# przemektmalon/SeqALib

Measured on AMD Instinct MI355X. Metric: GCUPS (DP cell updates/s) on batched 4k×4k SW; bit-exact score match, higher is better.
Workload: dtype f16 (integer-exact below 2048); 1 GPU; sw_batch_10000x4096x4096; pairs_per_gpu=10000, total_pairs=10000, m=4096, n=4096, algo=SmithWatermanSA, match=equal<char>, parallelism=pair-shard x1

## Files before the change

seqalib_amd/csrc/sa_traceback_so.hip:

```cpp
#include <limits.h>

#include "sa_internal.h"

namespace sa {

typedef const void __attribute__((address_space(1)))* so_gptr;
typedef void __attribute__((address_space(3)))* so_lptr;

constexpr int kSoOps = 64;
template <int R>
struct SoLds {
    static constexpr int RT = (2 * R + 31) / 32;
    static constexpr int kTags = 0;
    static constexpr int kEdge = kTags + 32 * RT * 256;
    static constexpr int kRowCodes = kEdge + 5 * 1024;
    static constexpr int kColCodes = kRowCodes + ((R + 3) / 4) * 256;
    static constexpr int kOps = kColCodes + 8 * 256;
    static constexpr int kBytes = kOps + kSoOps * 64;
};

__device__ __forceinline__ uint32_t so_code8(uint32_t sp, uint32_t b) {
    return (b == ((sp >> 8) & 255u) ? 8u : 0u) | (b == ((sp >> 16) & 255u) ? 16u : 0u) |
           (b == (sp >> 24) ? 24u : 0u);
}

template <int R>
__global__ __launch_bounds__(64) void traceback_so_kernel(TbParams P) {
    using L = SoLds<R>;
    constexpr int RT = L::RT;
    constexpr int BAND = kWave * R;
    __shared__ __attribute__((aligned(16))) uint8_t s_so[L::kBytes];
    typedef volatile uint8_t __attribute__((address_space(3))) lds_u8;
    typedef volatile uint32_t __attribute__((address_space(3))) lds_u32;
    typedef volatile uint16_t __attribute__((address_space(3))) lds_u16;
    lds_u8* const vb = (lds_u8*)s_so;
    lds_u32* const vw = (lds_u32*)s_so;
    const int lane = threadIdx.x;
    const uint32_t slot = blockIdx.x * blockDim.x + threadIdx.x;
    if (slot >= P.count) return;
    const uint32_t pidx = P.pair_base + slot;
    sa_result res = P.res[pidx];
    if (res.flags & SA_FLAG_BAD_SHAPE) return;
    if (!tb_mine(P, res.flags)) {
        tb_release(P, &P.res[pidx], res.flags);
        return;
    }
    res.flags &= tb_clear_mask(P);
    const uint64_t o1 = P.off1[pidx], o2 = P.off2[pidx];
    const int m = (int)(P.off1[pidx + 1] - o1);
    const int n = (int)(P.off2[pidx + 1] - o2);
    const uint8_t* s1 = P.seq1 + o1;
    const uint8_t* s2 = P.seq2 + o2;
    typedef uint8_t __attribute__((address_space(1))) glb_u8;
    glb_u8* ops = (glb_u8*)(P.ops + o1 + o2 + pidx);
    const uint8_t* const dir = P.dirs + (uint64_t)slot * P.dir_slot;
    const uint64_t band_stride = P.band_stride;
    const uint32_t npk = (uint32_t)(band_stride / (kWave * 16));
    const uint32_t* const sh_base = P.snap_h + (uint64_t)slot * P.snap_h_slot;
    const int32_t* const sp_base = P.snap_p + (uint64_t)slot * P.snap_p_slot;
    const uint32_t snap_nch = P.snap_nch;
    const uint32_t symp = P.prof[4];
    const uint32_t pf0 = P.prof[0], pf1 = P.prof[1], pf2 = P.prof[2], pf3 = P.prof[3];
    uint32_t mt = 0;
#pragma unroll
    for (int a = 0; a < 4; ++a)
#pragma unroll
        for (int b = 0; b < 4; ++b) {
            const uint32_t sa_ = (symp >> (8 * a)) & 255u, sb_ = (symp >> (8 * b)) & 255u;
            const bool v = P.lutbits ? ((P.lutbits[(sa_ << 3) | (sb_ >> 5)] >> (sb_ & 31u)) & 1u) != 0 : sa_ == sb_;
            mt |= (v ? 1u : 0u) << (a * 4 + b);
        }
    const bool allow = P.allow != 0;
    const int G = P.gap, MA = P.match, MI = P.mismatch;
    const uint32_t CU = (uint32_t)(-(4 * G + 2)) & 0xffffu;
    const uint32_t CL = (uint32_t)(4 * G + 1) & 0xffffu;

    uint32_t k = 0, k0 = 0;
    auto emit = [&](uint8_t op) __attribute__((always_inline)) {
        const uint32_t q = k - k0;
        vb[L::kOps + (q >> 2) * 256 + lane * 4 + (q & 3)] = op;
        ++k;
    };
    auto flush = [&]() __attribute__((always_inline)) {
        for (uint32_t q = 0; q < k - k0; ++q) ops[k0 + q] = vb[L::kOps + (q >> 2) * 256 + lane * 4 + (q & 3)];
        k0 = k;
    };

    int wb = -1, wt = 0, wc = 0;
    int cb = 0, ct = 0, cc = 0, cr = 0, cq = 0;
    auto locate = [&](int i, int j) __attribute__((always_inline)) {
        const int ii = i - 1;
        cb = ii / BAND;
        const int rem = ii - cb * BAND;
        ct = rem / R;
        cr = rem - ct * R;
        const int s = j - 1 + ct;
        cc = s >> 5;
        cq = s & 31;
    };
    auto ready = [&](int i, int j) __attribute__((always_inline)) -> bool {
        if (k - k0 >= (uint32_t)kSoOps) return false;
        if (!(i > 0 && j > 0)) return true;
        locate(i, j);
        return cb == wb && ct == wt && cc == wc;
    };
    auto recompute = [&](int i, int j) __attribute__((always_inline)) {
        if (!(i > 0 && j > 0)) return;
        locate(i, j);
        wb = cb; wt = ct; wc = cc;
        const int r0 = cb * BAND + ct * R;
        const int j0 = 32 * cc - ct;
        const bool has_top = !(cb == 0 && ct == 0);
        const int bp = ct > 0 ? cb : cb - 1, tp = ct > 0 ? ct - 1 : kWave - 1;
        const int slo = j0 + tp;
        const int pk0 = slo >> 3;
        if (has_top) {
            const uint8_t* base = dir + (uint64_t)bp * band_stride;
#pragma unroll
            for (int d = 0; d < 5; ++d) {
                const int pk = pk0 + d;
                if (pk >= 0 && (uint32_t)pk < npk)
                    __builtin_amdgcn_global_load_lds((so_gptr)(base + ((uint64_t)pk * kWave + tp) * 16),
                                                     (so_lptr)(s_so + L::kEdge + d * 1024), 16, 0, 0);
            }
        }
        int Hp[R];
        int corner = 0;
        const bool has_left = cc > 0 && j0 >= 1;
        if (has_left) {
            const uint64_t e = (uint64_t)cb * snap_nch + (cc - 1);
            const uint32_t* sh = sh_base + e * (R / 2) * kWave + ct;
#pragma unroll
            for (int q = 0; q < R / 2; ++q) {
                const uint32_t w = sh[q * kWave];
                Hp[2 * q] = (int)(w & 0xffffu) << 2;
                Hp[2 * q + 1] = (int)(w >> 16) << 2;
            }
            if (r0 > 0) corner = (sp_base[e * kWave + ct] & 0xffff) << 2;
        } else {
#pragma unroll
            for (int r = 0; r < R; ++r) Hp[r] = 0;
        }
        uint32_t tab[R];
#pragma unroll
        for (int r = 0; r < R; r += 4) {
            uint32_t cw = 0;
#pragma unroll
            for (int e = 0; e < 4 && r + e < R; ++e) {
                const int row = r0 + r + e;
                const uint32_t c8 = row < m ? so_code8(symp, s1[row]) : 0u;
                tab[r + e] = c8 == 0 ? pf0 : c8 == 8 ? pf1 : c8 == 16 ? pf2 : pf3;
                cw |= c8 << (8 * e);
            }
            vw[(L::kRowCodes >> 2) + (r >> 2) * 64 + lane] = cw;
        }
        const int qlo = j0 < 0 ? -j0 : 0;
        const int qhi = j - 1 - j0;
#pragma unroll
        for (int w = 0; w < 8; ++w) {
            uint32_t cw = 0;
#pragma unroll
            for (int e = 0; e < 4; ++e) {
                const int q = 4 * w + e, jj = j0 + q;
                cw |= (q >= qlo && q <= qhi && jj < n ? so_code8(symp, s2[jj]) : 0u) << (8 * e);
            }
            vw[(L::kColCodes >> 2) + w * 64 + lane] = cw;
        }
        asm volatile("s_waitcnt vmcnt(0)" ::: "memory");
        auto top_of = [&](int q) -> int {
            if (!has_top) return 0;
            const int s = slo + q;
            const int d = (s >> 3) - pk0;
            return (int)((lds_u16*)(s_so + L::kEdge + d * 1024 + lane * 16 + (s & 7) * 2))[0] << 2;
        };
        auto sym_of = [&](int q) -> uint32_t {
            return (vw[(L::kColCodes >> 2) + (q >> 2) * 64 + lane] >> (8 * (q & 3))) & 255u;
        };
        auto put = [&](int q, int r, uint32_t& rec) __attribute__((always_inline)) {
            if ((r & 15) == 15 || r == R - 1) {
                const uint32_t wv = (r & 15) == 15 ? rec : rec >> (32 - 2 * ((r & 15) + 1));
                vw[(q * RT + (r >> 4)) * 64 + lane] = wv;
                rec = 0;
            }
        };
#define SO_CELL(P, HP, HU, DR, REC, TAB, SYM)                                                      \
    "v_add_u16 %[" #P "0], %[cl], %[" HP "]\n\t"                                                  \
    "v_bfe_i32 %[" #P "dn], %[" TAB "], %[" SYM "], 8\n\t"                                         \
    "v_add_u16 %[" #P "dn], %[" HP "], %[" #P "dn]\n\t"                                            \
    "v_sub_u16_e64 %[" #P "1], %[" HU "], %[cu] clamp\n\t"                                         \
    "v_max_i16 %[" #P "0], %[" DR "], %[" #P "0]\n\t"                                              \
    "v_max_i16 %[" #P "0], %[" #P "1], %[" #P "0]\n\t"                                             \
    "v_and_b32 %[" HP "], -4, %[" #P "0]\n\t"                                                      \
    "v_alignbit_b32 %[" REC "], %[" #P "0], %[" REC "], 2\n\t"
#define SO_CELL2                                                                                   \
    "v_add_u16 %[a0], %[cl], %[ha]\n\t"                                                            \
    "v_add_u16 %[b0], %[cl], %[hb]\n\t"                                                            \
    "v_bfe_i32 %[adn], %[taba], %[syma], 8\n\t"                                                    \
    "v_bfe_i32 %[bdn], %[tabb], %[symb], 8\n\t"                                                    \
    "v_add_u16 %[adn], %[ha], %[adn]\n\t"                                                          \
    "v_add_u16 %[bdn], %[hb], %[bdn]\n\t"                                                          \
    "v_sub_u16_e64 %[a1], %[hb], %[cu] clamp\n\t"                                                  \
    "v_sub_u16_e64 %[b1], %[hub], %[cu] clamp\n\t"                                                 \
    "v_max_i16 %[a0], %[da], %[a0]\n\t"                                                            \
    "v_max_i16 %[b0], %[db], %[b0]\n\t"                                                            \
    "v_max_i16 %[a0], %[a1], %[a0]\n\t"                                                            \
    "v_max_i16 %[b0], %[b1], %[b0]\n\t"                                                            \
    "v_and_b32 %[ha], -4, %[a0]\n\t"                                                               \
    "v_and_b32 %[hb], -4, %[b0]\n\t"                                                               \
    "v_alignbit_b32 %[reca], %[a0], %[reca], 2\n\t"                                                \
    "v_alignbit_b32 %[recb], %[b0], %[recb], 2"
        auto column = [&](int q, int top, int ptop) __attribute__((always_inline)) {
            const uint32_t sym = sym_of(q);
            uint32_t dcur;
            asm("v_bfe_i32 %0, %1, %2, 8\n\tv_add_u16 %0, %3, %0" : "=&v"(dcur) : "v"(tab[0]), "v"(sym), "v"(ptop));
            uint32_t hu = (uint32_t)top, rec = 0;
#pragma unroll
            for (int r = 0; r < R; ++r) {
                uint32_t a0, a1, adn;
                asm(SO_CELL(a, "hp", "hu", "dr", "rec", "tabn", "sym")
                    : [a0] "=&v"(a0), [a1] "=&v"(a1), [adn] "=&v"(adn), [hp] "+v"(Hp[r]), [rec] "+v"(rec)
                    : [dr] "v"(dcur), [hu] "v"(hu), [cu] "s"(CU), [cl] "s"(CL),
                      [tabn] "v"(tab[r + 1 < R ? r + 1 : r]), [sym] "v"(sym));
                dcur = adn;
                hu = (uint32_t)Hp[r];
                put(q, r, rec);
            }
        };
        auto column_pair = [&](int q, int topA, int topB, int ptop) __attribute__((always_inline)) {
            const uint32_t symA = sym_of(q), symB = sym_of(q + 1);
            uint32_t da, db;
            asm("v_bfe_i32 %0, %1, %2, 8\n\tv_add_u16 %0, %3, %0" : "=&v"(da) : "v"(tab[0]), "v"(symA), "v"(ptop));
            asm("v_bfe_i32 %0, %1, %2, 8\n\tv_add_u16 %0, %3, %0" : "=&v"(db) : "v"(tab[0]), "v"(symB), "v"(topA));
            uint32_t recA = 0, recB = 0;
            {
                uint32_t a0, a1, adn;
                asm(SO_CELL(a, "hp", "hu", "dr", "rec", "tabn", "sym")
                    : [a0] "=&v"(a0), [a1] "=&v"(a1), [adn] "=&v"(adn), [hp] "+v"(Hp[0]), [rec] "+v"(recA)
                    : [dr] "v"(da), [hu] "v"((uint32_t)topA), [cu] "s"(CU), [cl] "s"(CL),
                      [tabn] "v"(tab[R > 1 ? 1 : 0]), [sym] "v"(symA));
                da = adn;
                put(q, 0, recA);
            }
#pragma unroll
            for (int r = 1; r < R; ++r) {
                const uint32_t hub = r >= 2 ? (uint32_t)Hp[r - 2] : (uint32_t)topB;
                uint32_t a0, a1, adn, b0, b1, bdn;
                asm(SO_CELL2
                    : [a0] "=&v"(a0), [a1] "=&v"(a1), [adn] "=&v"(adn), [b0] "=&v"(b0), [b1] "=&v"(b1),
                      [bdn] "=&v"(bdn), [ha] "+v"(Hp[r]), [hb] "+v"(Hp[r - 1]), [reca] "+v"(recA), [recb] "+v"(recB)
                    : [da] "v"(da), [db] "v"(db), [hub] "v"(hub), [cu] "s"(CU), [cl] "s"(CL),
                      [taba] "v"(tab[r + 1 < R ? r + 1 : r]), [syma] "v"(symA), [tabb] "v"(tab[r]), [symb] "v"(symB));
                da = adn;
                db = bdn;
                put(q, r, recA);
                put(q + 1, r - 1, recB);
            }
            {
                const uint32_t hub = R >= 2 ? (uint32_t)Hp[R - 2] : (uint32_t)topB;
                uint32_t b0, b1, bdn;
                asm(SO_CELL(b, "hp", "hu", "dr", "rec", "tabn", "sym")
                    : [b0] "=&v"(b0), [b1] "=&v"(b1), [bdn] "=&v"(bdn), [hp] "+v"(Hp[R - 1]), [rec] "+v"(recB)
                    : [dr] "v"(db), [hu] "v"(hub), [cu] "s"(CU), [cl] "s"(CL), [tabn] "v"(tab[R - 1]), [sym] "v"(symB));
                put(q + 1, R - 1, recB);
            }
        };
#undef SO_CELL
#undef SO_CELL2
        int ptop = corner;
        int q = qlo;
        for (; q + 1 <= qhi; q += 2) {
            const int ta = top_of(q), tb = top_of(q + 1);
            column_pair(q, ta, tb, ptop);
            ptop = tb;
        }
        if (q == qhi) column(q, top_of(q), ptop);
    };
    auto tag = [&]() __attribute__((always_inline)) -> uint32_t {
        return (vw[(cq * RT + (cr >> 4)) * 64 + lane] >> (2 * (cr & 15))) & 3u;
    };
    auto cell_match = [&]() __attribute__((always_inline)) -> bool {
        const uint32_t a = (vb[L::kRowCodes + (cr >> 2) * 256 + lane * 4 + (cr & 3)] >> 3) & 3u;
        const uint32_t b = (vb[L::kColCodes + (cq >> 2) * 256 + lane * 4 + (cq & 3)] >> 3) & 3u;
        return ((mt >> (a * 4 + b)) & 1u) != 0;
    };

    int i = res.end_i, j = res.end_j, V = res.score;
    if (m == 0 || n == 0) { i = 0; j = 0; }
    bool fin = false, parked = true;
    for (;;) {
        if (__builtin_amdgcn_ballot_w64(!fin && !parked) == 0) {
            if (__builtin_amdgcn_ballot_w64(!fin) == 0) break;
            if (!fin) { flush(); recompute(i, j); parked = false; }
        }
        if (!fin && !parked) {
            if (!(i > 0 && j > 0) || V == 0) {
                fin = true;
            } else if (!ready(i, j)) {
                parked = true;
            } else {
                const uint32_t f = tag();
                const bool dg = f == 3u, up = f == 2u;
                const bool v = dg && cell_match();
                emit(dg ? (v ? 'M' : (allow ? 'S' : 'X')) : (up ? 'U' : 'L'));
                V -= dg ? (v ? MA : MI) : G;
                i -= (dg || up) ? 1 : 0;
                j -= up ? 0 : 1;
            }
        }
    }
    flush();
    res.start_i = i;
    res.start_j = j;
    res.nops = k;
    P.res[pidx] = res;
}

constexpr int kSo4DefaultLp = 4;
#ifdef SA_TB_STATS
__device__ unsigned long long g_so4_stats[8];
extern "C" int sa_debug_so4_stats(unsigned long long* out, int reset) {
    if (hipMemcpyFromSymbol(out, HIP_SYMBOL(g_so4_stats), sizeof(g_so4_stats)) != hipSuccess) return 1;
    if (reset) {
        unsigned long long z[8] = {};
        if (hipMemcpyToSymbol(HIP_SYMBOL(g_so4_stats), z, sizeof(z)) != hipSuccess) return 1;
    }
    return 0;
}
#endif
template <int R, int LP>
struct So4Lds {
    static constexpr int kPairs = kWave / LP;
    static constexpr int kTags = 64;
    static constexpr int kQuad = 1024 + 32;
    static constexpr int kEdge = kTags + kPairs * kQuad;
    static constexpr int kEdge2 = kEdge + 64 * 16;
    static constexpr int kRowC = kEdge2 + (LP < 5 ? 64 * 16 : 0);
    static constexpr int kColC = kRowC + kPairs * 32;
    static constexpr int kBytes = kColC + kPairs * 32;
};

template <int ALG, int R, int LP>
__global__ __launch_bounds__(64) void traceback_so4_kernel(TbParams P) {
    constexpr bool NWK = ALG == SA_NW;
    using L = So4Lds<R, LP>;
    constexpr int RS = R / LP;
    constexpr int BAND = kWave * R;
    static_assert((LP == 4 || LP == 8) && R >= LP && R % LP == 0 && RS <= 16, "LP sublanes of <= 16 rows");
    __shared__ __attribute__((aligned(16))) uint8_t s_so[L::kBytes];
    typedef volatile uint8_t __attribute__((address_space(3))) lds_u8;
    typedef volatile uint32_t __attribute__((address_space(3))) lds_u32;
    typedef volatile uint16_t __attribute__((address_space(3))) lds_u16;
    typedef volatile uint64_t __attribute__((address_space(3))) lds_u64;
    lds_u8* const vb = (lds_u8*)s_so;
    lds_u32* const vw = (lds_u32*)s_so;
    const int lane = threadIdx.x, quad = lane / LP, sub = lane % LP;
    const uint32_t slot = blockIdx.x * L::kPairs + quad;
    bool live = slot < P.count;
    const uint32_t pidx = P.pair_base + (live ? slot : 0);
    sa_result res = P.res[pidx];
    if (live && !(res.flags & SA_FLAG_BAD_SHAPE) && !tb_mine(P, res.flags)) {
        if (sub == 0) tb_release(P, &P.res[pidx], res.flags);
        live = false;
    }
    live = live && !(res.flags & SA_FLAG_BAD_SHAPE);
    if (__builtin_amdgcn_ballot_w64(live) == 0) return;
    res.flags &= tb_clear_mask(P);
    const uint64_t o1 = P.off1[pidx], o2 = P.off2[pidx];
    const int m = (int)(P.off1[pidx + 1] - o1);
    const int n = (int)(P.off2[pidx + 1] - o2);
    const uint8_t* s1 = P.seq1 + o1;
    const uint8_t* s2 = P.seq2 + o2;
    typedef uint8_t __attribute__((address_space(1))) glb_u8;
    glb_u8* ops = (glb_u8*)(P.ops + o1 + o2 + pidx);
    const uint8_t* const dir = P.dirs + (uint64_t)(live ? slot : 0) * P.dir_slot;
    const uint64_t band_stride = P.band_stride;
    const uint32_t npk = (uint32_t)(band_stride / (kWave * 16));
    const uint32_t* const sh_base = P.snap_h + (uint64_t)(live ? slot : 0) * P.snap_h_slot;
    const int32_t* const sp_base = P.snap_p + (uint64_t)(live ? slot : 0) * P.snap_p_slot;
    const uint32_t snap_nch = P.snap_nch;
    const uint32_t symp = P.prof[4];
    const uint32_t pf0 = P.prof[0], pf1 = P.prof[1], pf2 = P.prof[2], pf3 = P.prof[3];
    uint32_t mt = 0;
#pragma unroll
    for (int a = 0; a < 4; ++a)
#pragma unroll
        for (int b = 0; b < 4; ++b) {
            const uint32_t sa_ = (symp >> (8 * a)) & 255u, sb_ = (symp >> (8 * b)) & 255u;
            const bool v = P.lutbits ? ((P.lutbits[(sa_ << 3) | (sb_ >> 5)] >> (sb_ & 31u)) & 1u) != 0 : sa_ == sb_;
            mt |= (v ? 1u : 0u) << (a * 4 + b);
        }
    const bool allow = P.allow != 0;
    const int G = P.gap, MA = P.match, MI = P.mismatch;
    const uint32_t CU = (uint32_t)(NWK ? 4 * G + 2 : -(4 * G + 2)) & 0xffffu;
    const uint32_t CL = (uint32_t)(4 * G + 1) & 0xffffu;
    const int D0 = P.t16_delta;
    auto border = [&](int x) __attribute__((always_inline)) -> int {
        return 4 * (x * G - D0);
    };

    uint32_t k = 0;
    auto emit = [&](uint8_t op) __attribute__((always_inline)) {
        if (sub == 0) ops[k] = op;
        ++k;
    };
    int cb = 0, ct = 0, cc = 0, cr = 0, cq = 0;
    auto locate = [&](int i, int j) __attribute__((always_inline)) {
        const int ii = i - 1;
        cb = ii / BAND;
        const int rem = ii - cb * BAND;
        ct = rem / R;
        cr = rem - ct * R;
        const int s = j - 1 + ct;
        cc = s >> 5;
        cq = s & 31;
    };
    uint64_t rowc = 0, colc = 0;
    auto pack_codes = [&](int base) __attribute__((always_inline)) -> uint64_t {
        uint64_t c = 0;
#pragma unroll
        for (int d = 0; d < 8; ++d) {
            uint32_t x = (vw[(base >> 2) + d] >> 3) & 0x03030303u;
            x = (x | (x >> 6)) & 0x000f000fu;
            x = (x | (x >> 12)) & 0xffu;
            c |= (uint64_t)x << (8 * d);
        }
        return c;
    };
#ifdef SA_TB_STATS
    unsigned long long st_rounds = 0, st_iters = 0, st_wait = 0, st_sub = 0, st_nsub = 0;
    const unsigned long long st_t0 = __builtin_amdgcn_s_memtime();
    unsigned long long st_a = 0;
#endif
    auto recompute = [&](bool act, int i, int j) __attribute__((always_inline)) {
#ifdef SA_TB_STATS
        st_a = __builtin_amdgcn_s_memtime();
#endif
        int r0 = 0, j0 = 0, qlo = 0, qhi = -1, slo = 0, pk0 = 0, bp = 0, tp = 0;
        bool has_top = false, has_left = false;
        if (act) {
            locate(i, j);
            r0 = cb * BAND + ct * R;
            j0 = 32 * cc - ct;
            qlo = j0 < 0 ? -j0 : 0;
            qhi = j - 1 - j0;
            has_top = !(cb == 0 && ct == 0);
            bp = ct > 0 ? cb : cb - 1;
            tp = ct > 0 ? ct - 1 : kWave - 1;
            slo = j0 + tp;
            pk0 = slo >> 3;
            has_left = cc > 0 && j0 >= 1;
            if (has_top) {
                const uint8_t* base = dir + (uint64_t)bp * band_stride;
                const int pk = pk0 + sub;
                if (sub < 5 && pk >= 0 && (uint32_t)pk < npk)
                    __builtin_amdgcn_global_load_lds((so_gptr)(base + ((uint64_t)pk * kWave + tp) * 16),
                                                     (so_lptr)(s_so + L::kEdge), 16, 0, 0);
                if constexpr (LP < 5) {
                    const int pk4 = pk0 + 4;
                    if (sub == 0 && pk4 >= 0 && (uint32_t)pk4 < npk)
                        __builtin_amdgcn_global_load_lds((so_gptr)(base + ((uint64_t)pk4 * kWave + tp) * 16),
                                                         (so_lptr)(s_so + L::kEdge2), 16, 0, 0);
                }
            }
        }
        int Hp[RS];
        int corner = 0;
        uint32_t tab[RS];
#pragma unroll
        for (int r = 0; r < RS; ++r) { Hp[r] = 0; tab[r] = pf0; }
        if (act) {
            const int rs0 = sub * RS;
            uint32_t w[RS], b1[RS], b2[32 / LP];
            const uint64_t e = has_left ? (uint64_t)cb * snap_nch + (cc - 1) : 0;
            const uint32_t* sh = sh_base + e * (R / 2) * kWave + ct;
#pragma unroll
            for (int r = 0; r < RS; ++r) w[r] = sh[((rs0 + r) >> 1) * kWave];
            const uint32_t wc = sh[(rs0 > 0 ? (rs0 - 1) >> 1 : 0) * kWave];
            const int32_t pc = sp_base[e * kWave + ct];
#pragma unroll
            for (int r = 0; r < RS; ++r) b1[r] = s1[min(r0 + rs0 + r, m - 1)];
#pragma unroll
            for (int x = 0; x < 32 / LP; ++x) b2[x] = s2[min(max(j0 + sub * (32 / LP) + x, 0), n - 1)];
            if constexpr (NWK) {
                if (!has_left) {
#pragma unroll
                    for (int r = 0; r < RS; ++r) Hp[r] = border(r0 + rs0 + r + 1);
                    corner = border(r0 + rs0);
                } else if (rs0 == 0 && r0 == 0) {
                    corner = border(j0);
                }
            }
            if (has_left) {
#pragma unroll
                for (int r = 0; r < RS; ++r) Hp[r] = (int)(((rs0 + r) & 1) ? (w[r] >> 16) : (w[r] & 0xffffu)) << 2;
                if (rs0 > 0) corner = (int)(((rs0 - 1) & 1) ? (wc >> 16) : (wc & 0xffffu)) << 2;
                else if (r0 > 0) corner = (pc & 0xffff) << 2;
            }
#pragma unroll
            for (int r = 0; r < RS; ++r) {
                const uint32_t c8 = r0 + rs0 + r < m ? so_code8(symp, b1[r]) : 0u;
                tab[r] = c8 == 0 ? pf0 : c8 == 8 ? pf1 : c8 == 16 ? pf2 : pf3;
                vb[L::kRowC + quad * 32 + rs0 + r] = (uint8_t)c8;
            }
#pragma unroll
            for (int x = 0; x < 32 / LP; ++x) {
                const int q = sub * (32 / LP) + x, jj = j0 + q;
                vb[L::kColC + quad * 32 + q] = (uint8_t)(q >= qlo && q <= qhi && jj < n ? so_code8(symp, b2[x]) : 0u);
            }
        }
        asm volatile("s_waitcnt vmcnt(0)" ::: "memory");
#ifdef SA_TB_STATS
        {
            const unsigned long long t = __builtin_amdgcn_s_memtime();
            st_wait += t - st_a;
            st_a = t;
        }
#endif
        if (act) colc = pack_codes(L::kColC + quad * 32);
        int hl = Hp[RS - 1];
        int prev_up = corner;
        int nmax = qhi - qlo + 1 + (LP - 1);
#pragma unroll
        for (int off = 32; off >= 1; off >>= 1) nmax = max(nmax, __shfl_xor(nmax, off));
        auto rd_top = [&](int q) __attribute__((always_inline)) -> int {
            const int s = slo + q;
            const int d = min(max((s >> 3) - pk0, 0), 4);
            const int off = (LP >= 5 || d < 4) ? L::kEdge + (quad * LP + d) * 16 : L::kEdge2 + quad * 64;
            const int v = (int)((lds_u16*)(s_so + off + (s & 7) * 2))[0] << 2;
            return has_top ? v : NWK ? border(j0 + q + 1) : 0;
        };
        int ntop = rd_top(qlo);
        for (int u = 0; u < nmax; ++u) {
            const int q = qlo + u - sub;
            const int top = ntop;
            ntop = rd_top(qlo + u + 1);
            const uint32_t sym = (uint32_t)((colc >> (2 * (q & 31))) & 3u) << 3;
            int up_h = LP == 4 ? __builtin_amdgcn_mov_dpp(hl, 0x90, 0xf, 0xf, false)
                               : __builtin_amdgcn_mov_dpp(hl, 0x111, 0xf, 0xf, false);
            const bool on = act && q >= qlo && q <= qhi;
            if (sub == 0) up_h = top;
            if (on) {
                uint32_t dcur;
                asm("v_bfe_i32 %0, %1, %2, 8\n\tv_add_u16 %0, %3, %0" : "=&v"(dcur) : "v"(tab[0]), "v"(sym), "v"(prev_up));
                uint32_t hu = (uint32_t)up_h;
                uint32_t rec[(RS + 3) / 4];
#pragma unroll
                for (int w = 0; w < (RS + 3) / 4; ++w) rec[w] = 0;
#pragma unroll
                for (int r = 0; r < RS; ++r) {
                    uint32_t a0, a1, adn;
                    const uint32_t kSel = (r % 4 == 0) ? 0x03020104u : (r % 4 == 1) ? 0x03020400u
                                            : (r % 4 == 2) ? 0x03040100u : 0x04020100u;
#define SO4_CELL(UP)                                                                               \
    asm("v_add_u16 %[a0], %[cl], %[hp]\n\t"                                                         \
        "v_bfe_i32 %[adn], %[tabn], %[sym], 8\n\t"                                                  \
        "v_add_u16 %[adn], %[hp], %[adn]\n\t" UP                                                   \
        "v_max_i16 %[a0], %[dr], %[a0]\n\t"                                                         \
        "v_max_i16 %[a0], %[a1], %[a0]\n\t"                                                         \
        "v_and_b32 %[hp], -4, %[a0]\n\t"                                                            \
        "v_perm_b32 %[rec], %[a0], %[rec], %[sel]"                                                 \
        : [a0] "=&v"(a0), [a1] "=&v"(a1), [adn] "=&v"(adn), [hp] "+v"(Hp[r]), [rec] "+v"(rec[r / 4]) \
        : [dr] "v"(dcur), [hu] "v"(hu), [cu] "s"(CU), [cl] "s"(CL),                                 \
          [tabn] "v"(tab[r + 1 < RS ? r + 1 : r]), [sym] "v"(sym), [sel] "s"(kSel))
                    if constexpr (NWK) SO4_CELL("v_add_u16 %[a1], %[cu], %[hu]\n\t");
                    else SO4_CELL("v_sub_u16_e64 %[a1], %[hu], %[cu] clamp\n\t");
#undef SO4_CELL
                    dcur = adn;
                    hu = (uint32_t)Hp[r];
                }
                const uint32_t tpo = (uint32_t)(L::kTags + quad * L::kQuad + q * 32 + sub * RS);
                if constexpr (RS == 1) vb[tpo] = (uint8_t)rec[0];
                else if constexpr (RS == 2) *(lds_u16*)(s_so + tpo) = (uint16_t)rec[0];
                else if constexpr (RS == 4) *(lds_u32*)(s_so + tpo) = rec[0];
                else if constexpr (RS == 8) *(lds_u64*)(s_so + tpo) = (uint64_t)rec[1] << 32 | rec[0];
                else {
#pragma unroll
                    for (int w = 0; w < RS / 4; ++w) ((lds_u32*)(s_so + tpo))[w] = rec[w];
                }
                prev_up = up_h;
                hl = Hp[RS - 1];
            }
        }
#ifdef SA_TB_STATS
        st_sub += __builtin_amdgcn_s_memtime() - st_a;
        st_nsub += (unsigned long long)nmax;
#endif
        if (act) rowc = pack_codes(L::kRowC + quad * 32);
    };

    int i = res.end_i, j = res.end_j, V = res.score;
    if (!NWK && (m == 0 || n == 0)) { i = 0; j = 0; }
    bool fin = !live, parked = true;
    const uint32_t tag_base = (uint32_t)(L::kTags + quad * L::kQuad);
    auto tag_at = [&](int r, int q) __attribute__((always_inline)) -> uint32_t {
        return (uint32_t)vb[tag_base + (uint32_t)q * 32u + (uint32_t)r] & 3u;
    };
    const int lead = quad * LP;
    for (;;) {
        i = __shfl(i, lead);
        j = __shfl(j, lead);
        fin = __shfl((int)fin, lead) != 0;
        parked = __shfl((int)parked, lead) != 0;
        if (__builtin_amdgcn_ballot_w64(!fin && !parked) == 0) {
            if (__builtin_amdgcn_ballot_w64(!fin) == 0) break;
#ifdef SA_TB_STATS
            ++st_rounds;
#endif
            recompute(!fin && i > 0 && j > 0, i, j);
            if (!fin) parked = false;
        }
        if (sub != 0 || fin || parked) continue;
        uint32_t f = tag_at(max(cr, 0), max(cq, 0));
        for (;;) {
#ifdef SA_TB_STATS
            ++st_iters;
#endif
            if (!((i > 0) & (j > 0) & (NWK | (V != 0)) & (cr >= 0) & (cq >= 0))) break;
            const uint32_t a3 = tag_base + (uint32_t)(cq * 32 + cr) - 33u;
            const uint32_t fd = (uint32_t)vb[a3] & 3u, fl = (uint32_t)vb[a3 + 1] & 3u, fu = (uint32_t)vb[a3 + 32] & 3u;
            const bool dg = f == 3u, up = f == 2u;
            const uint32_t ca = (uint32_t)(rowc >> (2 * cr)) & 3u, cb2 = (uint32_t)(colc >> (2 * cq)) & 3u;
            const bool v = dg & (((mt >> (ca * 4 + cb2)) & 1u) != 0);
            ops[k++] = dg ? (v ? 'M' : (allow ? 'S' : 'X')) : (up ? 'U' : 'L');
            V -= dg ? (v ? MA : MI) : G;
            const int di = (dg | up) ? 1 : 0, dj = up ? 0 : 1;
            i -= di;
            j -= dj;
            cr -= di;
            cq -= dj;
            f = dg ? fd : up ? fu : fl;
        }
        if (!((i > 0) & (j > 0) & (NWK | (V != 0)))) fin = true;
        else parked = true;
    }
#ifdef SA_TB_STATS
    if (lane == __builtin_amdgcn_readfirstlane(lane)) {
        atomicAdd(&g_so4_stats[0], st_rounds);
        atomicAdd(&g_so4_stats[1], st_iters);
        atomicAdd(&g_so4_stats[3], __builtin_amdgcn_s_memtime() - st_t0);
        atomicAdd(&g_so4_stats[4], st_wait);
        atomicAdd(&g_so4_stats[5], st_sub);
        atomicAdd(&g_so4_stats[6], st_nsub);
        atomicAdd(&g_so4_stats[7], 1ull);
    }
    if (live && sub == 0) atomicAdd(&g_so4_stats[2], (unsigned long long)k);
#endif
    if constexpr (NWK) {
        if (live) {
            for (; i > 0; --i) emit('U');
            for (; j > 0; --j) emit('L');
        }
    }
    if (live) {
        if (sub == 0) {
            res.start_i = i;
            res.start_j = j;
            res.nops = k;
            P.res[pidx] = res;
        }
    }
}

template <int ALG, int R>
__global__ __launch_bounds__(64) void traceback_soa_kernel(TbParams P) {
    constexpr int LP = 4, RS = R / LP, BAND = kWave * R;
    constexpr bool LG = ALG == SA_LOCAL_GOTOH;
    static_assert(R >= 4 && R <= 16 && R % LP == 0, "R in {4, 8, 16}");
    constexpr int kTags = 0, kEdge = kTags + 32 * 64 * 4, kRowC = kEdge + 3 * 1024, kColC = kRowC + 16 * 32;
    constexpr int kBytes = kColC + 16 * 32;
    __shared__ __attribute__((aligned(16))) uint8_t s_so[kBytes];
    typedef volatile uint8_t __attribute__((address_space(3))) lds_u8;
    typedef volatile uint32_t __attribute__((address_space(3))) lds_u32;
    lds_u8* const vb = (lds_u8*)s_so;
    lds_u32* const vw = (lds_u32*)s_so;
    const int lane = threadIdx.x, quad = lane / LP, sub = lane % LP;
    const uint32_t slot = blockIdx.x * (kWave / LP) + quad;
    bool live = slot < P.count;
    const uint32_t pidx = P.pair_base + (live ? slot : 0);
    sa_result res = P.res[pidx];
    if (live && !(res.flags & SA_FLAG_BAD_SHAPE) && !tb_mine(P, res.flags)) {
        if (sub == 0) tb_release(P, &P.res[pidx], res.flags);
        live = false;
    }
    live = live && !(res.flags & SA_FLAG_BAD_SHAPE);
    if (__builtin_amdgcn_ballot_w64(live) == 0) return;
    res.flags &= tb_clear_mask(P);
    uint32_t flags = res.flags;
    const uint64_t o1 = P.off1[pidx], o2 = P.off2[pidx];
    const int m = (int)(P.off1[pidx + 1] - o1);
    const int n = (int)(P.off2[pidx + 1] - o2);
    const uint8_t* s1 = P.seq1 + o1;
    const uint8_t* s2 = P.seq2 + o2;
    typedef uint8_t __attribute__((address_space(1))) glb_u8;
    glb_u8* ops = (glb_u8*)(P.ops + o1 + o2 + pidx);
    const uint8_t* const dir = P.dirs + (uint64_t)(live ? slot : 0) * P.dir_slot;
    const uint64_t band_stride = P.band_stride;
    const uint32_t npk = (uint32_t)(band_stride / (kWave * 16));
    const uint32_t* const sh_base = P.snap_h + (uint64_t)(live ? slot : 0) * P.snap_h_slot;
    const int32_t* const sp_base = P.snap_p + (uint64_t)(live ? slot : 0) * P.snap_p_slot;
    const uint32_t snap_nch = P.snap_nch;
    const uint32_t symp = P.prof[4];
    const uint32_t pf0 = P.prof[0], pf1 = P.prof[1], pf2 = P.prof[2], pf3 = P.prof[3];
    uint32_t mt = 0;
#pragma unroll
    for (int a = 0; a < 4; ++a)
#pragma unroll
        for (int b = 0; b < 4; ++b) {
            const uint32_t sa_ = (symp >> (8 * a)) & 255u, sb_ = (symp >> (8 * b)) & 255u;
            const bool v = P.lutbits ? ((P.lutbits[(sa_ << 3) | (sb_ >> 5)] >> (sb_ & 31u)) & 1u) != 0 : sa_ == sb_;
            mt |= (v ? 1u : 0u) << (a * 4 + b);
        }
    const bool allow = P.allow != 0;
    const int MA = P.match, MI = P.mismatch, GO = P.gap_open, GE = P.gap_extend, GOE = GO + GE;
    const int D0 = LG ? 0 : P.t16_delta;
    const int SENT = P.t16_sent;
    const uint32_t CXO = (uint32_t)(LG ? -(8 * GOE + 4) : 8 * GOE + 4) & 0xffffu;
    const uint32_t CXE = (uint32_t)(8 * GE + 1) & 0xffffu;
    const uint32_t CYO = (uint32_t)(8 * GOE + 2) & 0xffffu;
    auto mb = [&](int x) __attribute__((always_inline)) -> int { return LG ? 0 : 8 * ((x < 1 ? 0 : GO + x * GE) - D0); };

    uint32_t k = 0;
    auto emit = [&](uint8_t op) __attribute__((always_inline)) {
        if (sub == 0) ops[k] = op;
        ++k;
    };
    int cb = 0, ct = 0, cc = 0, cr = 0, cq = 0;
    auto locate = [&](int i, int j) __attribute__((always_inline)) {
        const int ii = i - 1;
        cb = ii / BAND;
        const int rem = ii - cb * BAND;
        ct = rem / R;
        cr = rem - ct * R;
        const int s = j - 1 + ct;
        cc = s >> 5;
        cq = s & 31;
    };
    auto recompute = [&](bool act, int i, int j) __attribute__((always_inline)) {
        int r0 = 0, j0 = 0, qlo = 0, qhi = -1, slo = 0, pk0 = 0, bp = 0, tp = 0;
        bool has_top = false, has_left = false;
        if (act) {
            locate(i, j);
            r0 = cb * BAND + ct * R;
            j0 = 32 * cc - ct;
            qlo = j0 < 0 ? -j0 : 0;
            qhi = j - 1 - j0;
            has_top = !(cb == 0 && ct == 0);
            bp = ct > 0 ? cb : cb - 1;
            tp = ct > 0 ? ct - 1 : kWave - 1;
            slo = j0 + tp;
            pk0 = slo >> 2;
            has_left = cc > 0 && j0 >= 1;
            if (has_top) {
                const uint8_t* base = dir + (uint64_t)bp * band_stride;
#pragma unroll
                for (int d = 0; d < 3; ++d) {
                    const int pk = pk0 + sub + 4 * d;
                    if (sub + 4 * d < 9 && pk >= 0 && (uint32_t)pk < npk)
                        __builtin_amdgcn_global_load_lds((so_gptr)(base + ((uint64_t)pk * kWave + tp) * 16),
                                                         (so_lptr)(s_so + kEdge + d * 1024), 16, 0, 0);
                }
            }
        }
        const int rs0 = sub * RS;
        int Mp[RS], Yp[RS];
        uint32_t tab[RS];
        int corner = 0;
#pragma unroll
        for (int r = 0; r < RS; ++r) { Mp[r] = 0; Yp[r] = SENT; tab[r] = pf0; }
        if (act) {
            if (has_left) {
                const uint64_t e = (uint64_t)cb * snap_nch + (cc - 1);
                const uint32_t* sh = sh_base + e * (R + 1) * kWave + ct;
#pragma unroll
                for (int r = 0; r < RS; ++r) {
                    const int rr = rs0 + r;
                    const uint32_t w = sh[(rr >> 1) * kWave], y = sh[(R / 2 + (rr >> 1)) * kWave];
                    const int mv = (int)((rr & 1) ? (w >> 16) : (w & 0xffffu));
                    const int bv = (int)(int16_t)((rr & 1) ? (y >> 16) : (y & 0xffffu));
                    Mp[r] = mv << 3;
                    Yp[r] = ((bv + GOE) << 3) + 2;
                }
                if (rs0 > 0) {
                    const uint32_t w = sh[((rs0 - 1) >> 1) * kWave];
                    corner = (int)(((rs0 - 1) & 1) ? (w >> 16) : (w & 0xffffu)) << 3;
                } else if (r0 > 0) {
                    corner = (sp_base[e * kWave + ct] & 0xffff) << 3;
                } else {
                    corner = mb(j0);
                }
            } else {
#pragma unroll
                for (int r = 0; r < RS; ++r) Mp[r] = mb(r0 + rs0 + r + 1);
                corner = mb(r0 + rs0);
            }
#pragma unroll
            for (int r = 0; r < RS; ++r) {
                const int row = r0 + rs0 + r;
                const uint32_t c8 = row < m ? so_code8(symp, s1[row]) : 0u;
                tab[r] = c8 == 0 ? pf0 : c8 == 8 ? pf1 : c8 == 16 ? pf2 : pf3;
                vb[kRowC + quad * 32 + rs0 + r] = (uint8_t)c8;
            }
#pragma unroll
            for (int e = 0; e < 32 / LP; ++e) {
                const int q = sub * (32 / LP) + e, jj = j0 + q;
                vb[kColC + quad * 32 + q] = (uint8_t)(q >= qlo && q <= qhi && jj < n ? so_code8(symp, s2[jj]) : 0u);
            }
        }
        asm volatile("s_waitcnt vmcnt(0)" ::: "memory");
        int hl = Mp[RS - 1], xl = SENT;
        int prev_up = corner;
        int nmax = qhi - qlo + 1 + (LP - 1);
#pragma unroll
        for (int off = 32; off >= 1; off >>= 1) nmax = max(nmax, __shfl_xor(nmax, off));
        for (int u = 0; u < nmax; ++u) {
            const int q = qlo + u - sub;
            const bool on = act && q >= qlo && q <= qhi;
            int up_h = __builtin_amdgcn_mov_dpp(hl, 0x90, 0xf, 0xf, false);
            int up_x = __builtin_amdgcn_mov_dpp(xl, 0x90, 0xf, 0xf, false);
            if (sub == 0) {
                up_h = 0;
                up_x = SENT;
                if (on) {
                    if (!has_top) {
                        up_h = mb(j0 + q + 1);
                    } else {
                        const int st = slo + q;
                        const int p = (st >> 2) - pk0;
                        const uint32_t w = vw[(kEdge >> 2) + (p >> 2) * 256 + (quad * LP + (p & 3)) * 4 + (st & 3)];
                        up_h = (int)(w & 0xffffu) << 3;
                        up_x = (((int)(int16_t)(w >> 16) + GOE) << 3) + 4;
                    }
                }
            }
            if (on) {
                const uint32_t sym = vb[kColC + quad * 32 + q];
                uint32_t dcur;
                asm("v_bfe_i32 %0, %1, %2, 8\n\tv_add_u16 %0, %3, %0" : "=&v"(dcur) : "v"(tab[0]), "v"(sym), "v"(prev_up));
                uint32_t hu = (uint32_t)up_h, xu = (uint32_t)up_x, rec = 0;
#pragma unroll
                for (int r = 0; r < RS; ++r) {
                    uint32_t t0, t1, xr, yr, dn;
                    const uint32_t tabn = tab[r + 1 < RS ? r + 1 : r];
                    if constexpr (LG) asm("v_sub_u16_e64 %[t0], %[hu], %[cxo] clamp" : [t0] "=v"(t0) : [hu] "v"(hu), [cxo] "s"(CXO));
                    else asm("v_add_u16 %[t0], %[cxo], %[hu]" : [t0] "=v"(t0) : [hu] "v"(hu), [cxo] "s"(CXO));
                    asm("v_add_u16 %[t1], %[cyo], %[hp]\n\t"
                        "v_add_u16 %[xr], %[cxe], %[xu]\n\t"
                        "v_add_u16 %[yr], %[cxe], %[yp]\n\t"
                        "v_max_i16 %[xr], %[t0], %[xr]\n\t"
                        "v_max_i16 %[yr], %[t1], %[yr]\n\t"
                        "v_bfe_i32 %[dn], %[tabn], %[sym], 8\n\t"
                        "v_add_u16 %[dn], %[hp], %[dn]\n\t"
                        "v_max_i16 %[t1], %[dr], %[xr]\n\t"
                        "v_max_i16 %[t1], %[yr], %[t1]"
                        : [t1] "=&v"(t1), [xr] "=&v"(xr), [yr] "=&v"(yr), [dn] "=&v"(dn)
                        : [t0] "v"(t0), [hp] "v"(Mp[r]), [xu] "v"(xu), [yp] "v"(Yp[r]), [dr] "v"(dcur),
                          [cxe] "s"(CXE), [cyo] "s"(CYO), [tabn] "v"(tabn), [sym] "v"(sym));
                    const uint32_t cls = (t1 >> 1) & 3u;
                    rec |= ((cls == 3u ? 8u : 0u) | (cls == 2u ? 4u : 0u) | ((xr & 1u) << 1) | (yr & 1u)) << (4 * r);
                    xu = xr & ~1u;
                    Yp[r] = (int)(yr & ~1u);
                    Mp[r] = (int)(t1 & ~7u);
                    hu = (uint32_t)Mp[r];
                    dcur = dn;
                }
                vw[q * 64 + lane] = rec;
                prev_up = up_h;
                hl = Mp[RS - 1];
                xl = (int)xu;
            }
        }
    };
    auto flag_of = [&](int r, int q) __attribute__((always_inline)) -> uint32_t {
        return (vw[q * 64 + quad * LP + r / RS] >> (4 * (r % RS))) & 15u;
    };
    auto match_of = [&](int r, int q) __attribute__((always_inline)) -> bool {
        const uint32_t a = (vb[kRowC + quad * 32 + r] >> 3) & 3u, b = (vb[kColC + quad * 32 + q] >> 3) & 3u;
        return ((mt >> (a * 4 + b)) & 1u) != 0;
    };

    int i, j, V = 0, st = 0;
    if constexpr (LG) { i = res.end_i; j = res.end_j; V = res.score; }
    else { i = m; j = n; }
    bool fin = !live, parked = true;
    for (;;) {
        if (__builtin_amdgcn_ballot_w64(!fin && !parked) == 0) {
            if (__builtin_amdgcn_ballot_w64(!fin) == 0) break;
            recompute(!fin, i, j);
            if (!fin) parked = false;
        }
        if (fin || parked) continue;
        if (!(i > 0 && j > 0)) { fin = true; continue; }
        if (LG && st == 0 && V <= 0) { fin = true; continue; }
        if (cr < 0 || cq < 0) { parked = true; continue; }
        const uint32_t f = flag_of(cr, cq);
        if (st == 0) {
            if (f & 8u) {
                const bool v = match_of(cr, cq);
                emit(v ? 'M' : (allow ? 'S' : 'X'));
                V -= v ? MA : MI;
                --i; --j; --cr; --cq;
            } else {
                st = (f & 4u) ? 1 : 2;
            }
        } else if (st == 1) {
            if constexpr (LG) {
                if (f & 2u) { emit('U'); V -= GE; --i; --cr; }
                else if (V > 0) { emit('U'); V -= GOE; --i; --cr; st = 0; }
                else if (V == 0) { emit('u'); fin = true; }
                else { flags |= SA_FLAG_DIVERGED; fin = true; }
            } else {
                emit('U'); --i; --cr;
                if (!(f & 2u)) st = 0;
            }
        } else {
            if constexpr (LG) {
                if (f & 1u) { emit('L'); V -= GE; --j; --cq; }
                else if (V > 0) { emit('L'); V -= GOE; --j; --cq; st = 0; }
                else if (V == 0) { emit('l'); fin = true; }
                else { flags |= SA_FLAG_DIVERGED; fin = true; }
            } else {
                emit('L'); --j; --cq;
                if (!(f & 1u)) st = 0;
            }
        }
    }
    if constexpr (!LG) {
        if (live) {
            for (; i > 0; --i) emit('U');
            for (; j > 0; --j) emit('L');
        }
    }
    if (live && sub == 0) {
        res.start_i = i;
        res.start_j = j;
        res.nops = k;
        res.flags = flags;
        P.res[pidx] = res;
    }
}

template <int ALG>
hipError_t launch_so4(int R, int lp, dim3 grid, dim3 block, const TbParams& p, hipStream_t stream) {
    if (lp == 8) {
        switch (R) {
            case 8: hipLaunchKernelGGL((traceback_so4_kernel<ALG, 8, 8>), grid, block, 0, stream, p); break;
            case 16: hipLaunchKernelGGL((traceback_so4_kernel<ALG, 16, 8>), grid, block, 0, stream, p); break;
            case 32: hipLaunchKernelGGL((traceback_so4_kernel<ALG, 32, 8>), grid, block, 0, stream, p); break;
            default: return hipErrorInvalidValue;
        }
        return hipGetLastError();
    }
    switch (R) {
        case 4: hipLaunchKernelGGL((traceback_so4_kernel<ALG, 4, 4>), grid, block, 0, stream, p); break;
        case 8: hipLaunchKernelGGL((traceback_so4_kernel<ALG, 8, 4>), grid, block, 0, stream, p); break;
        case 16: hipLaunchKernelGGL((traceback_so4_kernel<ALG, 16, 4>), grid, block, 0, stream, p); break;
        case 32: hipLaunchKernelGGL((traceback_so4_kernel<ALG, 32, 4>), grid, block, 0, stream, p); break;
        default: return hipErrorInvalidValue;
    }
    return hipGetLastError();
}

hipError_t launch_traceback_so(int algo, int R, const TbParams& p, hipStream_t stream) {
    const dim3 block(64);
    if (algo == SA_LOCAL_GOTOH || algo == SA_GLOBAL_GOTOH) {
        const dim3 grid((p.count + 15) / 16);
#define SA_TB_SOA(RR)                                                                                       \
    case RR:                                                                                                \
        if (algo == SA_LOCAL_GOTOH) hipLaunchKernelGGL((traceback_soa_kernel<SA_LOCAL_GOTOH, RR>), grid, block, 0, stream, p); \
        else hipLaunchKernelGGL((traceback_soa_kernel<SA_GLOBAL_GOTOH, RR>), grid, block, 0, stream, p);     \
        break;
        switch (R) {
            SA_TB_SOA(4)
            SA_TB_SOA(8)
            SA_TB_SOA(16)
            default: return hipErrorInvalidValue;
        }
#undef SA_TB_SOA
        return hipGetLastError();
    }
    if (algo != SA_SW && algo != SA_NW) return hipErrorInvalidValue;
    const char* e = getenv("SEQALIB_TB_SO");
    if (algo == SA_SW && e && e[0] == '1') {
        const dim3 grid((p.count + 63) / 64);
        switch (R) {
            case 4: hipLaunchKernelGGL(traceback_so_kernel<4>, grid, block, 0, stream, p); break;
            case 8: hipLaunchKernelGGL(traceback_so_kernel<8>, grid, block, 0, stream, p); break;
            case 16: hipLaunchKernelGGL(traceback_so_kernel<16>, grid, block, 0, stream, p); break;
            case 32: hipLaunchKernelGGL(traceback_so_kernel<32>, grid, block, 0, stream, p); break;
            default: return hipErrorInvalidValue;
        }
        return hipGetLastError();
    }
    int lp = p.so_lp == 8 && R >= 8 ? 8 : kSo4DefaultLp;
    if (const char* l = getenv("SEQALIB_TB_LP")) lp = (atoi(l) == 8 && R >= 8) ? 8 : 4;
    const uint32_t ppw = (uint32_t)(kWave / lp);
    const dim3 grid((p.count + ppw - 1) / ppw);
    return algo == SA_SW ? launch_so4<SA_SW>(R, lp, grid, block, p, stream) : launch_so4<SA_NW>(R, lp, grid, block, p, stream);
}

}
```

Baseline: 14130 GCUPS.

## Restage traceback column codes and top edges in LDS, branchless op emission

```diff
diff --git a/seqalib_amd/csrc/sa_traceback_so.hip b/seqalib_amd/csrc/sa_traceback_so.hip
--- a/seqalib_amd/csrc/sa_traceback_so.hip
+++ b/seqalib_amd/csrc/sa_traceback_so.hip
@@ -336,7 +336,11 @@
     static constexpr int kEdge2 = kEdge + 64 * 16;
     static constexpr int kRowC = kEdge2 + (LP < 5 ? 64 * 16 : 0);
     static constexpr int kColC = kRowC + kPairs * 32;
-    static constexpr int kBytes = kColC + kPairs * 32;
+    static constexpr int kTopW = LP == 4 ? 52 : 56;
+    static constexpr int kTopTail = 64;
+    static constexpr int kTop = kColC + kPairs * 32;
+    static constexpr int kBytes = kTop + (kPairs * kTopW + kTopTail) * 4;
+    static_assert(LP + 31 + 32 + LP + 1 < kTopW + kTopTail, "the last quad's read-ahead stays inside");
 };
 
 template <int ALG, int R, int LP>
@@ -350,9 +354,7 @@
     typedef volatile uint8_t __attribute__((address_space(3))) lds_u8;
     typedef volatile uint32_t __attribute__((address_space(3))) lds_u32;
     typedef volatile uint16_t __attribute__((address_space(3))) lds_u16;
-    typedef volatile uint64_t __attribute__((address_space(3))) lds_u64;
     lds_u8* const vb = (lds_u8*)s_so;
-    lds_u32* const vw = (lds_u32*)s_so;
     const int lane = threadIdx.x, quad = lane / LP, sub = lane % LP;
     const uint32_t slot = blockIdx.x * L::kPairs + quad;
     bool live = slot < P.count;
@@ -371,7 +373,10 @@
     const uint8_t* s1 = P.seq1 + o1;
     const uint8_t* s2 = P.seq2 + o2;
     typedef uint8_t __attribute__((address_space(1))) glb_u8;
-    glb_u8* ops = (glb_u8*)(P.ops + o1 + o2 + pidx);
+    const uint32_t pidx0 = P.pair_base + blockIdx.x * (uint32_t)L::kPairs;
+    const uint64_t obase = P.off1[pidx0] + P.off2[pidx0] + pidx0;
+    glb_u8* const ops = (glb_u8*)(P.ops + obase);
+    const uint32_t ooff = (uint32_t)(o1 + o2 + pidx - obase);
     const uint8_t* const dir = P.dirs + (uint64_t)(live ? slot : 0) * P.dir_slot;
     const uint64_t band_stride = P.band_stride;
     const uint32_t npk = (uint32_t)(band_stride / (kWave * 16));
@@ -389,8 +394,9 @@
             const bool v = P.lutbits ? ((P.lutbits[(sa_ << 3) | (sb_ >> 5)] >> (sb_ & 31u)) & 1u) != 0 : sa_ == sb_;
             mt |= (v ? 1u : 0u) << (a * 4 + b);
         }
-    const bool allow = P.allow != 0;
     const int G = P.gap, MA = P.match, MI = P.mismatch;
+    const uint32_t optab = 'L' | 'L' << 8 | 'U' << 16 | (uint32_t)(P.allow != 0 ? 'S' : 'X') << 24;
+    const uint32_t kOpM = (uint32_t)'M' - (optab >> 24);
     const uint32_t CU = (uint32_t)(NWK ? 4 * G + 2 : -(4 * G + 2)) & 0xffffu;
     const uint32_t CL = (uint32_t)(4 * G + 1) & 0xffffu;
     const int D0 = P.t16_delta;
@@ -400,7 +406,7 @@
 
     uint32_t k = 0;
     auto emit = [&](uint8_t op) __attribute__((always_inline)) {
-        if (sub == 0) ops[k] = op;
+        if (sub == 0) ops[ooff + k] = op;
         ++k;
     };
     int cb = 0, ct = 0, cc = 0, cr = 0, cq = 0;
@@ -413,18 +419,6 @@
         const int s = j - 1 + ct;
         cc = s >> 5;
         cq = s & 31;
-    };
-    uint64_t rowc = 0, colc = 0;
-    auto pack_codes = [&](int base) __attribute__((always_inline)) -> uint64_t {
-        uint64_t c = 0;
-#pragma unroll
-        for (int d = 0; d < 8; ++d) {
-            uint32_t x = (vw[(base >> 2) + d] >> 3) & 0x03030303u;
-            x = (x | (x >> 6)) & 0x000f000fu;
-            x = (x | (x >> 12)) & 0xffu;
-            c |= (uint64_t)x << (8 * d);
-        }
-        return c;
     };
 #ifdef SA_TB_STATS
     unsigned long long st_rounds = 0, st_iters = 0, st_wait = 0, st_sub = 0, st_nsub = 0;
@@ -465,9 +459,11 @@
         }
         int Hp[RS];
         int corner = 0;
-        uint32_t tab[RS];
+        uint32_t tab[RS], cw[32 / LP];
 #pragma unroll
         for (int r = 0; r < RS; ++r) { Hp[r] = 0; tab[r] = pf0; }
+#pragma unroll
+        for (int x = 0; x < 32 / LP; ++x) cw[x] = 0;
         if (act) {
             const int rs0 = sub * RS;
             uint32_t w[RS], b1[RS], b2[32 / LP];
@@ -500,15 +496,38 @@
             for (int r = 0; r < RS; ++r) {
                 const uint32_t c8 = r0 + rs0 + r < m ? so_code8(symp, b1[r]) : 0u;
                 tab[r] = c8 == 0 ? pf0 : c8 == 8 ? pf1 : c8 == 16 ? pf2 : pf3;
-                vb[L::kRowC + quad * 32 + rs0 + r] = (uint8_t)c8;
+                vb[L::kRowC + quad * 32 + rs0 + r] = (uint8_t)(c8 >> 1);
             }
 #pragma unroll
             for (int x = 0; x < 32 / LP; ++x) {
                 const int q = sub * (32 / LP) + x, jj = j0 + q;
-                vb[L::kColC + quad * 32 + q] = (uint8_t)(q >= qlo && q <= qhi && jj < n ? so_code8(symp, b2[x]) : 0u);
+                cw[x] = q >= qlo && q <= qhi && jj < n ? so_code8(symp, b2[x]) : 0u;
+                vb[L::kColC + quad * 32 + q] = (uint8_t)(cw[x] >> 3);
             }
         }
         asm volatile("s_waitcnt vmcnt(0)" ::: "memory");
+        if (act) {
+            constexpr int NX = 32 / LP;
+            const uint32_t wtop = (uint32_t)(L::kTop + (quad * L::kTopW + LP + sub * NX) * 4);
+            uint32_t e0, e1;
+            if constexpr (LP == 4) {
+                e0 = (uint32_t)(L::kEdge + lane * 16 + 14);
+                e1 = sub < 3 ? (uint32_t)(L::kEdge + (lane + 1) * 16) : (uint32_t)(L::kEdge2 + quad * 64);
+            } else {
+                const int s7 = sub * NX + 7;
+                e0 = (uint32_t)(L::kEdge + (quad * LP + (s7 >> 3)) * 16 + (s7 & 7) * 2);
+                e1 = (sub & 1) ? e0 + 2 : (uint32_t)(L::kEdge + (quad * LP + (s7 >> 3) + 1) * 16);
+            }
+            uint32_t ev[NX];
+#pragma unroll
+            for (int x = 0; x < NX; ++x) ev[x] = *(lds_u16*)(s_so + (x == 0 ? e0 : e1 + (uint32_t)(x - 1) * 2));
+#pragma unroll
+            for (int x = 0; x < NX; ++x) {
+                uint32_t top = ev[x] << 18;
+                if (!has_top) top = NWK ? (uint32_t)border(j0 + sub * NX + x + 1) << 16 : 0u;
+                *(lds_u32*)(s_so + wtop + x * 4) = cw[x] | top;
+            }
+        }
 #ifdef SA_TB_STATS
         {
             const unsigned long long t = __builtin_amdgcn_s_memtime();
@@ -516,66 +535,46 @@
             st_a = t;
         }
 #endif
-        if (act) colc = pack_codes(L::kColC + quad * 32);
         int hl = Hp[RS - 1];
         int prev_up = corner;
         int nmax = qhi - qlo + 1 + (LP - 1);
 #pragma unroll
         for (int off = 32; off >= 1; off >>= 1) nmax = max(nmax, __shfl_xor(nmax, off));
-        auto rd_top = [&](int q) __attribute__((always_inline)) -> int {
-            const int s = slo + q;
-            const int d = min(max((s >> 3) - pk0, 0), 4);
-            const int off = (LP >= 5 || d < 4) ? L::kEdge + (quad * LP + d) * 16 : L::kEdge2 + quad * 64;
-            const int v = (int)((lds_u16*)(s_so + off + (s & 7) * 2))[0] << 2;
-            return has_top ? v : NWK ? border(j0 + q + 1) : 0;
-        };
-        int ntop = rd_top(qlo);
-        for (int u = 0; u < nmax; ++u) {
-            const int q = qlo + u - sub;
-            const int top = ntop;
-            ntop = rd_top(qlo + u + 1);
-            const uint32_t sym = (uint32_t)((colc >> (2 * (q & 31))) & 3u) << 3;
+        const uint32_t ncol = (uint32_t)(qhi - qlo + 1);
+        uint32_t wa = (uint32_t)(L::kTop + (quad * L::kTopW + LP + qlo - sub) * 4);
+        uint32_t tpo = (uint32_t)(L::kTags + quad * L::kQuad + (qlo - sub) * 32 + sub * RS);
+        uint32_t wn = *(lds_u32*)(s_so + wa);
+        for (int u = 0; u < nmax; ++u, tpo += 32) {
+            const uint32_t sym = wn;
+            wa += 4;
+            wn = *(lds_u32*)(s_so + wa);
             int up_h = LP == 4 ? __builtin_amdgcn_mov_dpp(hl, 0x90, 0xf, 0xf, false)
                                : __builtin_amdgcn_mov_dpp(hl, 0x111, 0xf, 0xf, false);
-            const bool on = act && q >= qlo && q <= qhi;
-            if (sub == 0) up_h = top;
+            const bool on = (uint32_t)(u - sub) < ncol;
+            if (sub == 0) up_h = (int)(sym >> 16);
             if (on) {
                 uint32_t dcur;
                 asm("v_bfe_i32 %0, %1, %2, 8\n\tv_add_u16 %0, %3, %0" : "=&v"(dcur) : "v"(tab[0]), "v"(sym), "v"(prev_up));
                 uint32_t hu = (uint32_t)up_h;
-                uint32_t rec[(RS + 3) / 4];
-#pragma unroll
-                for (int w = 0; w < (RS + 3) / 4; ++w) rec[w] = 0;
 #pragma unroll
                 for (int r = 0; r < RS; ++r) {
                     uint32_t a0, a1, adn;
-                    const uint32_t kSel = (r % 4 == 0) ? 0x03020104u : (r % 4 == 1) ? 0x03020400u
-                                            : (r % 4 == 2) ? 0x03040100u : 0x04020100u;
 #define SO4_CELL(UP)                                                                               \
     asm("v_add_u16 %[a0], %[cl], %[hp]\n\t"                                                         \
         "v_bfe_i32 %[adn], %[tabn], %[sym], 8\n\t"                                                  \
         "v_add_u16 %[adn], %[hp], %[adn]\n\t" UP                                                   \
         "v_max_i16 %[a0], %[dr], %[a0]\n\t"                                                         \
         "v_max_i16 %[a0], %[a1], %[a0]\n\t"                                                         \
-        "v_and_b32 %[hp], -4, %[a0]\n\t"                                                            \
-        "v_perm_b32 %[rec], %[a0], %[rec], %[sel]"                                                 \
-        : [a0] "=&v"(a0), [a1] "=&v"(a1), [adn] "=&v"(adn), [hp] "+v"(Hp[r]), [rec] "+v"(rec[r / 4]) \
+        "v_and_b32 %[hp], -4, %[a0]"                                                                \
+        : [a0] "=&v"(a0), [a1] "=&v"(a1), [adn] "=&v"(adn), [hp] "+v"(Hp[r])                        \
         : [dr] "v"(dcur), [hu] "v"(hu), [cu] "s"(CU), [cl] "s"(CL),                                 \
-          [tabn] "v"(tab[r + 1 < RS ? r + 1 : r]), [sym] "v"(sym), [sel] "s"(kSel))
+          [tabn] "v"(tab[r + 1 < RS ? r + 1 : r]), [sym] "v"(sym))
                     if constexpr (NWK) SO4_CELL("v_add_u16 %[a1], %[cu], %[hu]\n\t");
                     else SO4_CELL("v_sub_u16_e64 %[a1], %[hu], %[cu] clamp\n\t");
 #undef SO4_CELL
+                    vb[tpo + r] = (uint8_t)a0;
                     dcur = adn;
                     hu = (uint32_t)Hp[r];
-                }
-                const uint32_t tpo = (uint32_t)(L::kTags + quad * L::kQuad + q * 32 + sub * RS);
-                if constexpr (RS == 1) vb[tpo] = (uint8_t)rec[0];
-                else if constexpr (RS == 2) *(lds_u16*)(s_so + tpo) = (uint16_t)rec[0];
-                else if constexpr (RS == 4) *(lds_u32*)(s_so + tpo) = rec[0];
-                else if constexpr (RS == 8) *(lds_u64*)(s_so + tpo) = (uint64_t)rec[1] << 32 | rec[0];
-                else {
-#pragma unroll
-                    for (int w = 0; w < RS / 4; ++w) ((lds_u32*)(s_so + tpo))[w] = rec[w];
                 }
                 prev_up = up_h;
                 hl = Hp[RS - 1];
@@ -585,13 +584,13 @@
         st_sub += __builtin_amdgcn_s_memtime() - st_a;
         st_nsub += (unsigned long long)nmax;
 #endif
-        if (act) rowc = pack_codes(L::kRowC + quad * 32);
     };
 
     int i = res.end_i, j = res.end_j, V = res.score;
     if (!NWK && (m == 0 || n == 0)) { i = 0; j = 0; }
     bool fin = !live, parked = true;
     const uint32_t tag_base = (uint32_t)(L::kTags + quad * L::kQuad);
+    const uint32_t rowc_base = (uint32_t)(L::kRowC + quad * 32), colc_base = (uint32_t)(L::kColC + quad * 32);
     auto tag_at = [&](int r, int q) __attribute__((always_inline)) -> uint32_t {
         return (uint32_t)vb[tag_base + (uint32_t)q * 32u + (uint32_t)r] & 3u;
     };
@@ -611,6 +610,7 @@
         }
         if (sub != 0 || fin || parked) continue;
         uint32_t f = tag_at(max(cr, 0), max(cq, 0));
+        uint32_t ca = vb[rowc_base + (uint32_t)max(cr, 0)], cb2 = vb[colc_base + (uint32_t)max(cq, 0)];
         for (;;) {
 #ifdef SA_TB_STATS
             ++st_iters;
@@ -618,17 +618,18 @@
             if (!((i > 0) & (j > 0) & (NWK | (V != 0)) & (cr >= 0) & (cq >= 0))) break;
             const uint32_t a3 = tag_base + (uint32_t)(cq * 32 + cr) - 33u;
             const uint32_t fd = (uint32_t)vb[a3] & 3u, fl = (uint32_t)vb[a3 + 1] & 3u, fu = (uint32_t)vb[a3 + 32] & 3u;
-            const bool dg = f == 3u, up = f == 2u;
-            const uint32_t ca = (uint32_t)(rowc >> (2 * cr)) & 3u, cb2 = (uint32_t)(colc >> (2 * cq)) & 3u;
-            const bool v = dg & (((mt >> (ca * 4 + cb2)) & 1u) != 0);
-            ops[k++] = dg ? (v ? 'M' : (allow ? 'S' : 'X')) : (up ? 'U' : 'L');
-            V -= dg ? (v ? MA : MI) : G;
-            const int di = (dg | up) ? 1 : 0, dj = up ? 0 : 1;
-            i -= di;
-            j -= dj;
-            cr -= di;
-            cq -= dj;
-            f = dg ? fd : up ? fu : fl;
+            const uint32_t cap = vb[rowc_base + (uint32_t)cr - 1u], cbp = vb[colc_base + (uint32_t)cq - 1u];
+            const uint32_t di = f >> 1, dg = f & di, dj = (di ^ dg) ^ 1u;
+            const uint32_t vm = dg & (mt >> (ca | cb2));
+            ops[ooff + k++] = (uint8_t)((optab >> (8 * f)) + vm * kOpM);
+            V -= G + __mul24((int)dg, MI - G) + __mul24((int)vm, MA - MI);
+            i -= (int)di;
+            j -= (int)dj;
+            cr -= (int)di;
+            cq -= (int)dj;
+            f = dg ? fd : di ? fu : fl;
+            ca = di ? cap : ca;
+            cb2 = dj ? cbp : cb2;
         }
         if (!((i > 0) & (j > 0) & (NWK | (V != 0)))) fin = true;
         else parked = true;
```

New measurement: 14400 GCUPS (median of 6 runs). +1.9%, better.
